# mittagessen/conformer_ocr

Measured on AMD Instinct MI355X. Metric: text lines/sec (whole node) + CER vs reference, 96×1200 bf16 batch, higher is better.
Workload: dtype bf16; 1 GPU; cfg2: conformer D=256 L=12 heads=4 sub_ch=256, batch 32 x 96x1200 per GPU, forward + CTC greedy; batches_in_queue=1, parallelism=1 independent rank(s), weights by one RCCL broadcast, streams_per_gpu=4, hipgraph_replay=True, launched_by=in-process, gpu_max_hw_queues=4, gpu_max_hw_queues_preset_by_caller=True

## Files before the change

### conformer_ocr_amd/build.py

```python
from __future__ import annotations

import os
import shutil
import subprocess
import sys

PKG = os.path.dirname(os.path.abspath(__file__))
CSRC = os.path.join(PKG, 'csrc')
LIB_DIR = os.path.join(PKG, 'lib')
LIB = os.path.join(LIB_DIR, 'libcocr_hip.so')
INCLUDE = os.path.join(os.path.dirname(PKG), 'include')
ARCH = 'gfx950'


def sources():
    srcs = [os.path.join(CSRC, f) for f in sorted(os.listdir(CSRC))]
    return srcs + [os.path.join(INCLUDE, 'cocr.h')]


def source_hash() -> str:
    import hashlib
    h = hashlib.sha256()
    for s in sources():
        h.update(os.path.basename(s).encode() + b'\0')
# ... 27 lines not shown
        i = cmd.index('-amdgpu-mfma-vgpr-form')
        cmd = cmd[:i - 1] + cmd[i + 1:]
        if verbose:
            print('retrying without -amdgpu-mfma-vgpr-form', flush=True)
        subprocess.check_call(cmd)


def build(force: bool = False, verbose: bool = True, out: str = None) -> str:
    if out is not None:
        return _build_to(out, verbose)
    if not force and up_to_date():
        return LIB
    return _build_to(LIB, verbose)


def _build_to(LIB: str, verbose: bool) -> str:
    hipcc = shutil.which('hipcc') or '/opt/rocm/bin/hipcc'
    if not os.path.exists(hipcc):
        raise RuntimeError('hipcc not found: cannot build libcocr_hip.so')
    os.makedirs(LIB_DIR, exist_ok=True)
    src_hash = source_hash()
    obj_dir = os.path.join(LIB_DIR, 'obj', src_hash)
    os.makedirs(obj_dir, exist_ok=True)
    flags = [f'--offload-arch={ARCH}', '-O3', '-std=c++17', '-fPIC', '-fno-gpu-rdc', '-mllvm', '-amdgpu-mfma-vgpr-form',
             '-Wall', '-Wno-unused-function', f'-DCOCR_SRC_HASH="{src_hash}"', '-I', INCLUDE]
    flags[0:0] = os.environ.get('COCR_HIPCC_FLAGS', '').split()
    units = [f for f in sorted(os.listdir(CSRC)) if f.endswith('.hip')]
    objs = [os.path.join(obj_dir, u[:-4] + '.o') for u in units]
    jobs = [([hipcc] + flags + ['-c', os.path.join(CSRC, u), '-o', o], verbose) for u, o in zip(units, objs)]
    from concurrent.futures import ThreadPoolExecutor
    with ThreadPoolExecutor(max_workers=min(len(jobs), os.cpu_count() or 1)) as pool:
        list(pool.map(_compile, jobs))
    link = [hipcc, f'--offload-arch={ARCH}', '-shared', '-fPIC', '-fno-gpu-rdc'] + objs + ['-o', LIB + '.tmp']
    if verbose:
        print(' '.join(link), flush=True)
    subprocess.check_call(link)
    os.replace(LIB + '.tmp', LIB)
    with open(LIB + '.srchash.tmp', 'w') as fp:
        fp.write(src_hash + '\n')
    os.replace(LIB + '.srchash.tmp', LIB + '.srchash')
    for d in os.listdir(os.path.join(LIB_DIR, 'obj')):
# ... 9 lines not shown
```

### conformer_ocr_amd/csrc/attention.hip.h

```cpp
#pragma once
#include "common.hip.h"

__device__ __forceinline__ int xcd_remap_i(int bid, int nwg) {
    const int q = nwg >> 3, r = nwg & 7, xcd = bid & 7;
    return (xcd < r ? xcd * (q + 1) : r * (q + 1) + (xcd - r) * q) + (bid >> 3);
}

__device__ __forceinline__ float max3_f(float a, float b, float c) {
    float r;
    asm("v_max3_f32 %0, %1, %2, %3" : "=v"(r) : "v"(a), "v"(b), "v"(c));
    return r;
}

#define COCR_MFMA_WAIT "s_nop 7\n\ts_nop 7\n\ts_nop 3"
__device__ __forceinline__ void mfma_results_fence(f32x4 (&a)[4]) { asm volatile(COCR_MFMA_WAIT : "+v"(a[0]), "+v"(a[1]), "+v"(a[2]), "+v"(a[3])); }
__device__ __forceinline__ void mfma_results_fence(f32x4 (&a)[4], f32x4 (&b)[4]) {
    asm volatile(COCR_MFMA_WAIT : "+v"(a[0]), "+v"(a[1]), "+v"(a[2]), "+v"(a[3]), "+v"(b[0]), "+v"(b[1]), "+v"(b[2]), "+v"(b[3]));
}
__device__ __forceinline__ void mfma_results_fence(f32x4 (&a)[4], f32x4 (&b)[4], f32x4 (&c)[4]) {
    asm volatile(COCR_MFMA_WAIT : "+v"(a[0]), "+v"(a[1]), "+v"(a[2]), "+v"(a[3]), "+v"(b[0]), "+v"(b[1]), "+v"(b[2]), "+v"(b[3]), "+v"(c[0]), "+v"(c[1]), "+v"(c[2]),
                 "+v"(c[3]));
}

#ifndef COCR_ATT_EXP
// ... 421 lines not shown
constexpr int AF_SK = 20;
#ifndef COCR_AF_TWOPART
#define COCR_AF_TWOPART 1
#endif
constexpr int AF_WAVES = 8;
constexpr int AF_SROWS = 32;
constexpr size_t AF_LDS = (size_t)(2 * AF_TK + 16 * AF_QT + AF_TK) * 128 + AF_WAVES * AF_SROWS * AF_SK * sizeof(float);
static_assert(AF_LDS <= 160 * 1024, "LDS of the resident attention kernel");

struct AttnFullState {
    bf16x8 qu[2][2], qv[2][2];
    f32x4 o[2][4], osum[2];
    float m_run[2];
};

template <int NT>
__device__ __forceinline__ void attn_full_tiles(const unsigned char *ks, const unsigned char *vs, const unsigned char *ps, float *sk,
                                                AttnFullState &st, int lb_first, int Tn, int Tk, int kg0, int lane, bool sync_after_first = false) {
    typedef bf16_t T;
    constexpr int KC = 2, DT = 4, RS = 128;
    const int il = lane & 15, g = lane >> 4;
    const int fo0 = ((g ^ (il & 7)) << 4), fo1 = (((4 + g) ^ (il & 7)) << 4);
    auto &qu = st.qu;
    auto &qv = st.qv;
    auto &o = st.o;
    auto &osum = st.osum;
    auto &m_run = st.m_run;
    bf16x8 ones;
#pragma unroll
    for (int j = 0; j < 8; ++j) ones[j] = il == 0 ? (T)1.0f : (T)0.0f;
// ... 83 lines not shown
#pragma unroll
        for (int t = 0; t < NT; ++t) { const float x = __shfl_xor(tmax[t], 16, 64); tmax[t] = max3_f(tmax[t], x, x); }
#pragma unroll
        for (int t = 0; t < NT; ++t) { const float x = __shfl_xor(tmax[t], 32, 64); tmax[t] = max3_f(tmax[t], x, x); }
        constexpr float LAZY = 8.0f;
        bool need[NT], any = first_tile;
#pragma unroll
        for (int t = 0; t < NT; ++t) { need[t] = first_tile || __builtin_amdgcn_ballot_w64(tmax[t] > LAZY) != 0; any = any || need[t]; }
        if (any) {
#pragma unroll
            for (int t = 0; t < NT; ++t) {
                const float delta = first_tile ? tmax[t] : (need[t] ? fmaxf(tmax[t], 0.f) : 0.f);
                const float alpha = first_tile ? 1.0f : __builtin_amdgcn_exp2f(-delta);
                m_run[t] = first_tile ? tmax[t] : m_run[t] + delta;
#pragma unroll
                for (int r = 0; r < 4; ++r) osum[t][r] *= alpha;
#pragma unroll
                for (int d = 0; d < DT; ++d)
#pragma unroll
                    for (int r = 0; r < 4; ++r) o[t][d][r] *= alpha;
#pragma unroll
                for (int tt = 0; tt < 4; ++tt)
#pragma unroll
                    for (int r = 0; r < 4; ++r) sc[t][tt][r] -= delta;
            }
        }
#pragma unroll
        for (int t = 0; t < NT; ++t) {
#pragma unroll
            for (int tt = 0; tt < 4; ++tt)
#pragma unroll
                for (int r = 0; r < 4; ++r) pb[t][tt >> 1][4 * (tt & 1) + r] = (T)__builtin_amdgcn_exp2f(sc[t][tt][r]);
            osum[t] = mma16(ones, pb[t][0], osum[t]);
            osum[t] = mma16(ones, pb[t][1], osum[t]);
        }
#pragma unroll
        for (int d = 0; d < DT; ++d) {
            const bf16x8 v0 = load_vt_frag<true>(vs, RS, j0, d, il, g, T()), v1 = load_vt_frag<true>(vs, RS, j0 + 32, d, il, g, T());
#pragma unroll
// ... 146 lines not shown
```

### conformer_ocr_amd/csrc/common.hip.h

```cpp
#pragma once
#include <hip/hip_runtime.h>
#include <stdint.h>

typedef __attribute__((address_space(3))) void *lds_ptr_t;
typedef __attribute__((address_space(1))) const void *gbl_ptr_t;

typedef __bf16 bf16_t;
typedef __bf16 bf16x8 __attribute__((ext_vector_type(8)));
typedef __bf16 bf16x4 __attribute__((ext_vector_type(4)));
typedef __bf16 bf16x2 __attribute__((ext_vector_type(2)));
typedef float f32x2 __attribute__((ext_vector_type(2)));
typedef float f32x4 __attribute__((ext_vector_type(4)));
typedef float f32x8 __attribute__((ext_vector_type(8)));

#define COCR_WAVE 64

template <typename T> struct FragOf;
template <> struct FragOf<bf16_t> { typedef bf16x8 type; };
template <> struct FragOf<float> { typedef f32x8 type; };

__device__ __forceinline__ f32x4 mma16(const bf16x8 &a, const bf16x8 &b, f32x4 c) {
    return __builtin_amdgcn_mfma_f32_16x16x32_bf16(a, b, c, 0, 0, 0);
}
__device__ __forceinline__ f32x4 mma16(const f32x8 &a, const f32x8 &b, f32x4 c) {
// ... 9 lines not shown
}
template <typename T> __device__ __forceinline__ typename FragOf<T>::type zero_frag() {
    typename FragOf<T>::type z;
#pragma unroll
    for (int j = 0; j < 8; ++j) z[j] = (T)0.0f;
    return z;
}

__device__ __forceinline__ float to_f32(float x) { return x; }
__device__ __forceinline__ float to_f32(bf16_t x) { return (float)x; }
template <typename T> __device__ __forceinline__ T from_f32(float x) { return (T)x; }

__device__ __forceinline__ float sigmoid_f(float x) { return __builtin_amdgcn_rcpf(1.0f + __expf(-x)); }
__device__ __forceinline__ float silu_f(float x) { return x * sigmoid_f(x); }

template <int CTRL, int ROW_MASK> __device__ __forceinline__ float dpp_f32(float v, float old) {
    return __builtin_bit_cast(float, __builtin_amdgcn_update_dpp(__builtin_bit_cast(int, old), __builtin_bit_cast(int, v), CTRL, ROW_MASK, 0xF, false));
}
__device__ __forceinline__ float wave_sum(float v) {
    v += dpp_f32<0xB1, 0xF>(v, 0.f);
    v += dpp_f32<0x4E, 0xF>(v, 0.f);
    v += dpp_f32<0x141, 0xF>(v, 0.f);
    v += dpp_f32<0x140, 0xF>(v, 0.f);
    v += dpp_f32<0x142, 0xA>(v, 0.f);
    v += dpp_f32<0x143, 0xC>(v, 0.f);
    return __builtin_bit_cast(float, __builtin_amdgcn_readlane(__builtin_bit_cast(int, v), 63));
}
__device__ __forceinline__ float wave_max(float v) {
    v = fmaxf(v, dpp_f32<0xB1, 0xF>(v, v));
    v = fmaxf(v, dpp_f32<0x4E, 0xF>(v, v));
// ... 10 lines not shown
```

### conformer_ocr_amd/csrc/rowchain.hip.h

```cpp
#pragma once
#include <type_traits>

#include "gemm.hip.h"
#include "rowchain_args.hip.h"

#ifndef COCR_STAMP_WG
#define COCR_STAMP_WG 7
#endif
#ifndef COCR_RC_EXP
#define COCR_RC_EXP 0
#endif

__device__ __forceinline__ void swap32(float &a, float &b) { asm("s_nop 1\n\tv_permlane32_swap_b32 %0, %1" : "+v"(a), "+v"(b)); }
__device__ __forceinline__ void swap16(float &a, float &b) { asm("s_nop 1\n\tv_permlane16_swap_b32 %0, %1" : "+v"(a), "+v"(b)); }
__device__ __forceinline__ float butterfly4(float a, float b, float c, float d) {
    swap32(a, b);
    swap32(c, d);
    float ab = a + b, cd = c + d;
    swap16(ab, cd);
    return ab + cd;
}

__device__ __forceinline__ int xcd_remap_rows(int bid, int nwg) {
    const int q = nwg >> 3, r = nwg & 7, xcd = bid & 7;
    return (xcd < r ? xcd * (q + 1) : r * (q + 1) + (xcd - r) * q) + (bid >> 3);
}

#ifndef COCR_RC_PAIR
#define COCR_RC_PAIR 0
#endif
template <int D, int MT> constexpr bool rowchain_pair_form() { return COCR_RC_PAIR && D == 256 && MT == 3; }

template <int D, int MT> constexpr size_t rowchain_slack_bytes() { return rowchain_pair_form<D, MT>() ? 2048 : 4096; }
template <int D, int MT> constexpr size_t rowchain_lds_bytes() {
    return (size_t)(D / 64) * 16 * MT * 128 + 2 * 4 * (size_t)(16 * MT) * 128 + rowchain_slack_bytes<D, MT>() + 16 * (size_t)D + 12 * (size_t)(16 * MT) + 64;
}
template <int D, int MT> constexpr int rowchain_dw_pass() { return rowchain_pair_form<D, MT>() ? 128 : 256; }
template <int D, int MT, int DWK> constexpr int rowchain_taps_place() {
    if (DWK == 0 || (DWK + 1) % 8 != 0) return 0;
    constexpr size_t cw = rowchain_dw_pass<D, MT>(), rpi = 64 / (cw / 8);
    constexpr size_t hsb = 2 * 4 * (size_t)(16 * MT) * 128 + rowchain_slack_bytes<D, MT>(), win = ((16 * MT + DWK - 1 + rpi - 1) / rpi) * 1024, taps = (size_t)(DWK + 1) * cw * 4;
    if (win + taps <= hsb) return 1;
    if (rowchain_pair_form<D, MT>()) return 0;
    if (rowchain_lds_bytes<D, MT>() + taps <= 160 * 1024) return 2;
// ... 20 lines not shown
    constexpr int PANEL = BMC * 128;
    constexpr int IMGX = (D / 64) * PANEL;
    constexpr int IMGH = 4 * PANEL;
    constexpr int OS = 256 * 2 + 16;
    constexpr int OSD = D * 2 + 16;
    constexpr int SLICE = 16 * 512;
    constexpr int PROW = 80;
    constexpr int HSB = 2 * IMGH + (int)rowchain_slack_bytes<D, MT>();
    extern __shared__ __attribute__((aligned(16))) unsigned char smem[];
    unsigned char *xa = smem;
    unsigned char *hs = smem + IMGX;
    float *lnp = reinterpret_cast<float *>(smem + IMGX + HSB);
    long long *rowoff = reinterpret_cast<long long *>(smem + IMGX + HSB + 16 * D);
    int *tpos = reinterpret_cast<int *>(smem + IMGX + HSB + 16 * D + 8 * BMC);

    const int tid = threadIdx.x, lane = tid & 63;
    const int wave = __builtin_amdgcn_readfirstlane(tid >> 6);
    const int r16 = lane & 15, g = lane >> 4, swz = r16 & 7;
    const int rblk = p.xcd_order ? xcd_remap_rows(blockIdx.x, gridDim.x) : (int)blockIdx.x;
    const int M = p.M, m0 = rblk * BMC, mend = min(M, m0 + BMC);
    const int lrow = lane >> 3, cpos = lane & 7;
#ifdef COCR_CHAIN_STAMPS_BUILD
    int sk = 0;
#define RSTAMP() { if (p.stamps && rblk == COCR_STAMP_WG && lane == 0) p.stamps[wave * 64 + sk] = __builtin_readcyclecounter(); ++sk; }
#else
#define RSTAMP()
#endif
    RSTAMP()
    auto lds_fence_barrier = [&]() {
        asm volatile("s_waitcnt lgkmcnt(0)" ::: "memory");
// ... 68 lines not shown
    };
    RSTAMP()
    dw_taps(0);
    RSTAMP()
    constexpr int RING = rowchain_pair_form<D, MT>() ? 8 : 16;
    bf16x8 ring[RING];
    auto fill = [&](const T *slice, int f) { ring[f % RING] = *reinterpret_cast<const bf16x8 *>(slice + f * 512 + lane * 8); };
    const T *cur_run = p.st[0].W + (size_t)wave * (FRONT0 ? p.st[0].K / 256 : KS) * SLICE;
    {
#pragma unroll
        for (int f = 0; f < RING; ++f) fill(cur_run, f);
    }
    __builtin_amdgcn_sched_barrier(0);
    RSTAMP()
    f32x4 xs[MT][NJ];
    const size_t xblk = ((size_t)rblk * 8 + wave) * (MT * NJ) * 256 + lane * 4;
    auto load_stream = [&]() {
        if (p.x_in_blocked) {
#pragma unroll
            for (int i = 0; i < MT; ++i)
#pragma unroll
                for (int c = 0; c < NJ; ++c) {
                    if constexpr (COCR_RC_EXP & 1) xs[i][c] = (f32x4){(float)r16, 1.f, (float)g, 0.5f};
                    else xs[i][c] = *reinterpret_cast<const f32x4 *>(p.x + xblk + (i * NJ + c) * 256);
                }
            return;
        }
#pragma unroll
        for (int i = 0; i < MT; ++i) {
            const float *xrow = p.x + (size_t)min(m0 + 16 * i + r16, mend - 1) * D + 32 * wave + 4 * g;
#pragma unroll
            for (int c = 0; c < NJ; ++c) {
                if constexpr (COCR_RC_EXP & 1) xs[i][c] = (f32x4){(float)r16, 1.f, (float)g, 0.5f};
                else xs[i][c] = *reinterpret_cast<const f32x4 *>(xrow + 256 * (c >> 1) + 16 * (c & 1));
            }
        }
    };
    constexpr int EARLY_XS = (DWK == 0 && !FRONT0) ? MT * NJ : 0;
    if constexpr (DWK == 0 && !FRONT0) load_stream();
    __builtin_amdgcn_sched_barrier(0);
    if (tid < BMC) {
        const int m = min(m0 + tid, M - 1), b = m / p.T_, t = m - b * p.T_;
        rowoff[tid] = ((long long)b * p.heads * p.Tp + t) * p.dhp;
        tpos[tid] = t;
    }
// ... 73 lines not shown
                        }
                    }
                }
#pragma unroll
                for (int i = 0; i < G; ++i) {
                    const int row = rb + i, cc = h * CW + c;
                    const bf16x2 o = (COCR_RC_EXP & 16384) ? (bf16x2){(T)acc[i][0], (T)acc[i][1]} : (bf16x2){(T)silu_f(acc[i][0]), (T)silu_f(acc[i][1])};
                    *reinterpret_cast<bf16x2 *>(xa + (cc >> 6) * PANEL + row * 128 + ((((cc & 63) >> 3) ^ (row & 7)) << 4) + (cc & 7) * 2) = o;
                    if constexpr (TAPS) {
                        if (p.tap_dw && m0 + row < mend) *reinterpret_cast<bf16x2 *>(p.tap_dw + (size_t)(m0 + row) * D + cc) = o;
                    }
                }
            }
            lds_fence_barrier();
        }
        load_stream();
        __builtin_amdgcn_sched_barrier(0);
        RSTAMP()
    }

    auto step = [&](const unsigned char *img, auto &acc, int c0, const T *nxt, auto &&side, auto FRESH, auto KKC) {
        constexpr bool fresh = decltype(FRESH)::value;
        constexpr int KK = decltype(KKC)::value;
#pragma unroll
        for (int kk = 0; kk < KK; ++kk) {
            constexpr int HT = MT > 3 ? MT / 2 : MT;
#pragma unroll
            for (int h0 = 0; h0 < MT; h0 += HT) {
                bf16x8 a[HT];
#pragma unroll
                for (int i = 0; i < HT; ++i) {
// ... 21 lines not shown
                    fill(nxt, 2 * (kk & 3));
                    fill(nxt, 2 * (kk & 3) + 1);
                }
            }
            side(kk);
            __builtin_amdgcn_sched_barrier(0);
        }
        if constexpr (KK < (RING == 16 ? 8 : 4) && !(COCR_RC_EXP & 128)) {
#pragma unroll
            for (int f = 2 * KK; f < RING; ++f) fill(nxt, f);
            __builtin_amdgcn_sched_barrier(0);
        }
        cur_run = nxt;
    };
    auto no_side = [](int) {};
    auto request_ln_params = [&](const ChainStage &st) {
        if (wave < 4) {
            const float *src = wave == 0 ? st.g1 : wave == 1 ? st.b1 : wave == 2 ? (st.g2 ? st.g2 : st.g1) : (st.b2 ? st.b2 : st.b1);
#pragma unroll
            for (int c = 0; c < D / 256; ++c)
                __builtin_amdgcn_global_load_lds((gbl_ptr_t)(src + c * 256 + lane * 4), (lds_ptr_t)(reinterpret_cast<unsigned char *>(lnp) + wave * D * 4 + c * 1024), 16, 0, 0);
        }
    };
    struct Bias2 { f32x4 v[2]; };
    auto load_bias = [&](const float *bias) {
        Bias2 b;
        b.v[0] = *reinterpret_cast<const f32x4 *>(bias + 32 * wave + 4 * g);
        b.v[1] = *reinterpret_cast<const f32x4 *>(bias + 32 * wave + 16 + 4 * g);
        return b;
    };
    auto add_bias_to_stream = [&](const float *bias, float alpha) {
#pragma unroll
        for (int ns = 0; ns < NS; ++ns) {
            const Bias2 b = load_bias(bias + 256 * ns);
#pragma unroll
            for (int j = 0; j < 2; ++j)
#pragma unroll
                for (int i = 0; i < MT; ++i) xs[i][2 * ns + j] += b.v[j] * alpha;
        }
    };
    auto store_stream = [&](float *dst) {
        if constexpr (COCR_RC_EXP & 2) { asm volatile("" :: "v"(xs[0][0][0])); return; }
        if (dst == p.x && p.x_out_blocked) {
#pragma unroll
            for (int i = 0; i < MT; ++i)
#pragma unroll
                for (int c = 0; c < NJ; ++c) *reinterpret_cast<f32x4 *>(dst + xblk + (i * NJ + c) * 256) = xs[i][c];
            return;
        }
#pragma unroll
        for (int i = 0; i < MT; ++i) {
            if (m0 + 16 * i + r16 < mend) {
                float *xrow = dst + (size_t)(m0 + 16 * i + r16) * D + 32 * wave + 4 * g;
#pragma unroll
                for (int c = 0; c < NJ; ++c) *reinterpret_cast<f32x4 *>(xrow + 256 * (c >> 1) + 16 * (c & 1)) = xs[i][c];
            }
        }
    };
    auto row_stats = [&](unsigned char *pbuf, bool wait_params, float (&mean)[MT], float (&rstd)[MT]) {
        if constexpr (COCR_RC_EXP & 32) { for (int i = 0; i < MT; ++i) { mean[i] = 0.f; rstd[i] = 1.f; } lds_fence_barrier(); return; }
        float s[MT], ss[MT];
#pragma unroll
        for (int i = 0; i < MT; ++i) {
            f32x4 a = xs[i][0], b = xs[i][0] * xs[i][0];
#pragma unroll
            for (int c = 1; c < NJ; ++c) { a += xs[i][c]; b = __builtin_elementwise_fma(xs[i][c], xs[i][c], b); }
            s[i] = (a[0] + a[1]) + (a[2] + a[3]);
            ss[i] = (b[0] + b[1]) + (b[2] + b[3]);
        }
#pragma unroll
        for (int i0 = 0; i0 < MT; i0 += 4) {
            const int i1 = min(i0 + 1, MT - 1), i2 = min(i0 + 2, MT - 1), i3 = min(i0 + 3, MT - 1);
            const float ts = butterfly4(s[i0], s[i1], s[i2], s[i3]), tss = butterfly4(ss[i0], ss[i1], ss[i2], ss[i3]);
            const int tile = g == 0 ? i0 : g == 1 ? i2 : g == 2 ? i1 : i3;
            *reinterpret_cast<f32x2 *>(pbuf + (16 * tile + r16) * PROW + wave * 8) = (f32x2){ts, tss};
        }
        if (wait_params && wave < 4) {
            if constexpr (KD == 8 && KL == 8) asm volatile("s_waitcnt vmcnt(%0)" :: "n"(RING) : "memory");
            else asm volatile("s_waitcnt vmcnt(0)" ::: "memory");
        }
        lds_fence_barrier();
        const float inv_d = p.inv_d;
#pragma unroll
        for (int i = 0; i < MT; ++i) {
            const unsigned char *pr = pbuf + (16 * i + r16) * PROW;
            f32x4 v = *reinterpret_cast<const f32x4 *>(pr);
            if constexpr (!(COCR_RC_EXP & 4)) {
#pragma unroll
                for (int w2 = 1; w2 < 4; ++w2) v += *reinterpret_cast<const f32x4 *>(pr + 16 * w2);
            }
            const float S = v[0] + v[2], SS = v[1] + v[3];
            mean[i] = S * inv_d;
            const float ex2 = SS * inv_d;
            rstd[i] = __builtin_amdgcn_rsqf(fmaxf(__builtin_fmaf(-mean[i], mean[i], ex2), 0.f) + 1e-5f);
        }
    };
    auto normalise = [&](int which, const float (&mean)[MT], const float (&rstd)[MT], auto IN_PLACE) {
        constexpr bool in_place = decltype(IN_PLACE)::value;
        if constexpr (COCR_RC_EXP & 8192) return;
        const float *ga = lnp + which * 2 * D, *be = ga + D;
#pragma unroll
        for (int c = 0; c < NJ; ++c) {
            const int col = 256 * (c >> 1) + 32 * wave + 16 * (c & 1) + 4 * g;
            const f32x4 gv = *reinterpret_cast<const f32x4 *>(ga + col), bv = *reinterpret_cast<const f32x4 *>(be + col);
#pragma unroll
            for (int i = 0; i < MT; ++i) {
                const float r = rstd[i], mr = -mean[i] * r;
                const f32x4 y = __builtin_elementwise_fma(__builtin_elementwise_fma(xs[i][c], (f32x4){r, r, r, r}, (f32x4){mr, mr, mr, mr}), gv, bv);
                if constexpr (in_place) {
                    xs[i][c] = y;
                } else {
                    const int row = 16 * i + r16;
                    const bf16x4 o = {(T)y[0], (T)y[1], (T)y[2], (T)y[3]};
                    *reinterpret_cast<bf16x4 *>(xa + (col >> 6) * PANEL + row * 128 + ((((col & 63) >> 3) ^ (row & 7)) << 4) + (col & 4) * 2) = o;
                }
            }
        }
    };
    auto rowln_epilogue = [&](const ChainStage &st, unsigned char *pbuf) {
        const bool chained = st.g2 != nullptr;
        if constexpr (TAPS) { if (st.tap_pre) store_stream(st.tap_pre); }
        float mean[MT], rstd[MT];
        if (!chained) {
            if (st.store_x) store_stream(p.x);
            row_stats(pbuf, true, mean, rstd);
            normalise(0, mean, rstd, std::false_type{});
        } else {
            row_stats(pbuf, true, mean, rstd);
            normalise(0, mean, rstd, std::true_type{});
            if (st.store_x) store_stream(p.x);
            if constexpr (TAPS) { if (st.tap_post) store_stream(st.tap_post); }
            row_stats(pbuf + BMC * PROW, false, mean, rstd);
            normalise(1, mean, rstd, std::false_type{});
        }
        lds_fence_barrier();
        if (st.store_xn) {
            for (int id = tid; id < BMC * (D / 8); id += 512) {
                const int row = id / (D / 8), ch = id - row * (D / 8);
                if (m0 + row < mend)
                    copy16(p.xn + (size_t)(m0 + row) * D + ch * 8, reinterpret_cast<const T *>(xa + (ch >> 3) * PANEL + row * 128 + (((ch & 7) ^ (row & 7)) << 4)));
            }
        }
    };

    auto run_stage = [&](auto KIND, auto FIRST, const ChainStage &st, const T *after) {
        constexpr int kind = decltype(KIND)::value;
        if constexpr (kind == ST_ROWLN) {
            request_ln_params(st);
            auto slice = [&](int ns, int ks) { return st.W + ((size_t)(ns * 8 + wave) * KS + ks) * SLICE; };
            if constexpr (decltype(FIRST)::value) {
                f32x4 acc[MT][NJ];
#pragma unroll
                for (int ns = 0; ns < NS; ++ns)
#pragma unroll
                    for (int ks = 0; ks < KS; ++ks) {
                        const T *nxt = ks + 1 < KS ? slice(ns, ks + 1) : (ns + 1 < NS ? slice(ns + 1, 0) : after);
                        if (ks == 0) step(xa, acc, 2 * ns, nxt, no_side, std::true_type{}, KKR{});
                        else step(xa + ks * 4 * PANEL, acc, 2 * ns, nxt, no_side, std::false_type{}, KKR{});
                    }
                add_bias_to_stream(st.bias, 1.0f);
#pragma unroll
                for (int i = 0; i < MT; ++i)
#pragma unroll
                    for (int c = 0; c < NJ; ++c) xs[i][c] += acc[i][c];
            } else {
                add_bias_to_stream(st.bias, 1.0f);
#pragma unroll
                for (int ns = 0; ns < NS; ++ns)
#pragma unroll
                    for (int ks = 0; ks < KS; ++ks)
                        step(xa + ks * 4 * PANEL, xs, 2 * ns, ks + 1 < KS ? slice(ns, ks + 1) : (ns + 1 < NS ? slice(ns + 1, 0) : after), no_side, std::false_type{}, KKR{});
            }
            RSTAMP()
            rowln_epilogue(st, hs);
            RSTAMP()
        } else if constexpr (kind == ST_FRONT) {
            static_assert(decltype(FIRST)::value, "FRONT is a first stage");
            request_ln_params(st);
            const int nsl = st.K / 256;
            auto slice = [&](int ns, int ks) { return st.W + ((size_t)(ns * 8 + wave) * nsl + ks) * SLICE; };
#pragma unroll
            for (int i = 0; i < MT; ++i)
#pragma unroll
                for (int c = 0; c < NJ; ++c) xs[i][c] = (f32x4){0.f, 0.f, 0.f, 0.f};
            add_bias_to_stream(st.bias, 1.0f);
#pragma unroll 1
            for (int ks = 0; ks < nsl; ++ks) {
                if (ks + 1 < nsl) front_dma(ks + 1);
                const unsigned char *img = hs + (ks & 1) * IMGH;
#pragma unroll
                for (int ns = 0; ns < NS; ++ns)
                    step(img, xs, 2 * ns, ns + 1 < NS ? slice(ns + 1, ks) : (ks + 1 < nsl ? slice(0, ks + 1) : after), no_side, std::false_type{}, KK8{});
                if (ks + 1 < nsl) {
                    asm volatile("s_waitcnt vmcnt(%0)" :: "n"(RING) : "memory");
                    lds_fence_barrier();
                }
            }
            RSTAMP()
            rowln_epilogue(st, hs + (nsl & 1) * IMGH);
            RSTAMP()
        } else if constexpr (kind == ST_FFN) {
            const int FF = st.N, nchunks = FF / 256;
            auto w1 = [&](int c, int ks) { return st.W + ((size_t)(c * 8 + wave) * KS + ks) * SLICE; };
            auto w2 = [&](int c, int ns) { return st.W2 + ((size_t)(ns * 8 + wave) * (FF / 32) + c * 8) * 1024; };
            f32x4 acc1[MT][2];
            Bias2 bb;
            auto silu_tile = [&](int tIdx, unsigned char *hb, auto PIN) {
                if constexpr (COCR_RC_EXP & 4096) return;
                const int i = tIdx >> 1, j = tIdx & 1;
                if constexpr (decltype(PIN)::value) asm volatile("" : "+v"(acc1[i][j]));
                const int jj = 32 * wave + 16 * j + 4 * g;
                const int ch16 = (jj & 63) >> 3, row = 16 * i + r16;
                typedef float f32x2_t __attribute__((ext_vector_type(2)));
                const f32x4 v4 = acc1[i][j] + bb.v[j];
                unsigned packed[2];
#pragma unroll
                for (int h = 0; h < 2; ++h) {
                    const f32x2_t v = {v4[2 * h], v4[2 * h + 1]};
                    f32x2_t e = v * (f32x2_t){-1.44269504088896340736f, -1.44269504088896340736f};
                    if constexpr (!(COCR_RC_EXP & 16)) e = (f32x2_t){__builtin_amdgcn_exp2f(e[0]), __builtin_amdgcn_exp2f(e[1])} + (f32x2_t){1.0f, 1.0f};
                    const f32x2_t o = (COCR_RC_EXP & 16) ? v * e : v * (f32x2_t){__builtin_amdgcn_rcpf(e[0]), __builtin_amdgcn_rcpf(e[1])};
                    packed[h] = __builtin_bit_cast(unsigned, __builtin_convertvector(o, bf16x2));
                }
                typedef unsigned u32x2_t __attribute__((ext_vector_type(2)));
                *reinterpret_cast<u32x2_t *>(hb + (jj >> 6) * PANEL + row * 128 + ((ch16 ^ (row & 7)) << 4) + ((jj & 7) >> 2) * 8) = (u32x2_t){packed[0], packed[1]};
            };
            auto p1 = [&](int c, const T *then) {
                if (wave >= 4) __builtin_amdgcn_s_setprio(1);
#pragma unroll
                for (int ks = 0; ks < KS; ++ks) {
                    if (ks == 0) step(xa, acc1, 0, KS > 1 ? w1(c, 1) : then, no_side, std::true_type{}, KKP1{});
                    else step(xa + ks * 4 * PANEL, acc1, 0, ks + 1 < KS ? w1(c, ks + 1) : then, no_side, std::false_type{}, KKP1{});
                }
                if (wave >= 4) __builtin_amdgcn_s_setprio(0);
            };
            request_ln_params(st);
            bb = load_bias(st.bias);
            p1(0, nchunks > 1 ? w1(1, 0) : w2(0, 0));
            RSTAMP()
#pragma unroll
            for (int t2 = 0; t2 < 2 * MT; ++t2) silu_tile(t2, hs, std::false_type{});
            add_bias_to_stream(st.bias2, st.alpha);
            RSTAMP()
            lds_fence_barrier();
            RSTAMP()
            for (int c = 1; c < nchunks; ++c) {
                bb = load_bias(st.bias + c * 256);
                p1(c, w2(c - 1, 0));
                RSTAMP()
                unsigned char *hb = hs + (c & 1) * IMGH;
#pragma unroll
                for (int ns = 0; ns < NS; ++ns)
                    step(hs + ((c - 1) & 1) * IMGH, xs, 2 * ns, ns + 1 < NS ? w2(c - 1, ns + 1) : (c + 1 < nchunks ? w1(c + 1, 0) : w2(c, 0)),
                         [&](int kk) {
#pragma unroll
                             for (int t2 = 0; t2 < 2 * MT; ++t2) if ((t2 * 8 * NS) / (2 * MT) == ns * 8 + kk) silu_tile(t2, hb, std::true_type{});
                         }, std::false_type{}, KK8{});
                RSTAMP()
                lds_fence_barrier();
                RSTAMP()
            }
#pragma unroll
            for (int ns = 0; ns < NS; ++ns)
                step(hs + ((nchunks - 1) & 1) * IMGH, xs, 2 * ns, ns + 1 < NS ? w2(nchunks - 1, ns + 1) : after, no_side, std::false_type{}, KKL{});
            RSTAMP()
            rowln_epilogue(st, hs + (nchunks & 1) * IMGH);
            RSTAMP()
        } else if constexpr (kind == ST_GLU) {
            EpiGLU<T> e{st.out, D, st.bias, 2 * D};
            auto slice = [&](int s2, int ks) { return st.W + ((size_t)(s2 * 8 + wave) * KS + ks) * SLICE; };
            constexpr int NSTEP = 2 * D / 256;
#pragma unroll 1
            for (int s2 = 0; s2 < NSTEP; ++s2) {
                const Bias2 bb = load_bias(st.bias + s2 * 256);
                f32x4 acc[MT][2];
#pragma unroll
                for (int ks = 0; ks < KS; ++ks) {
                    const T *nxt = ks + 1 < KS ? slice(s2, ks + 1) : (s2 + 1 < NSTEP ? slice(s2 + 1, 0) : after);
                    if (ks == 0) step(xa, acc, 0, nxt, no_side, std::true_type{}, KKG{});
                    else step(xa + ks * 4 * PANEL, acc, 0, nxt, no_side, std::false_type{}, KKG{});
                }
#pragma unroll
                for (int i = 0; i < MT; ++i) {
                    const int row = 16 * i + r16;
                    bf16x4 o;
#pragma unroll
                    for (int q = 0; q < 4; ++q) o[q] = (T)((acc[i][0][q] + bb.v[0][q]) * sigmoid_f(acc[i][1][q] + bb.v[1][q]));
                    *reinterpret_cast<bf16x4 *>(hs + row * OSD + (s2 * 128 + 16 * wave + 4 * g) * 2) = o;
                }
            }
            lds_fence_barrier();
            for (int id = tid; id < BMC * (D / 8); id += 512) {
                const int row = id / (D / 8), ch = id - row * (D / 8);
                if (m0 + row < mend) e.store(m0 + row, ch * 8, reinterpret_cast<const T *>(hs + row * OSD + ch * 16), 8);
            }
        } else if constexpr (kind == ST_QKV) {
            auto slice = [&](int s3, int ks) { return st.W + ((size_t)(s3 * 8 + wave) * KS + ks) * SLICE; };
            constexpr int NSTEP = 3 * D / 256;
#pragma unroll
            for (int s3 = 0; s3 < NSTEP; ++s3) {
                const Bias2 bb = load_bias(st.bias + s3 * 256);
                f32x4 acc[MT][2];
#pragma unroll
                for (int ks = 0; ks < KS; ++ks) {
                    const T *nxt = ks + 1 < KS ? slice(s3, ks + 1) : (s3 + 1 < NSTEP ? slice(s3 + 1, 0) : after);
                    if (ks == 0) step(xa, acc, 0, nxt, no_side, std::true_type{}, KKQ{});
                    else step(xa + ks * 4 * PANEL, acc, 0, nxt, no_side, std::false_type{}, KKQ{});
                }
                unsigned char *tile = hs + (s3 & 1) * (BMC * OS);
                if constexpr (COCR_RC_EXP & 1024) { asm volatile("" :: "v"(acc[0][0]), "v"(acc[MT - 1][1])); continue; }
#pragma unroll
                for (int j = 0; j < 2; ++j)
#pragma unroll
                    for (int i = 0; i < MT; ++i) {
                        const int row = 16 * i + r16;
                        bf16x4 o;
#pragma unroll
                        for (int q = 0; q < 4; ++q) o[q] = (T)(acc[i][j][q] + bb.v[j][q]);
                        *reinterpret_cast<bf16x4 *>(tile + row * OS + (32 * wave + 16 * j + 4 * g) * 2) = o;
                    }
                RSTAMP()
                lds_fence_barrier();
                {
                    const int which = s3 / NS;
                    T *base = which == 0 ? st.q : (which == 1 ? st.k : st.v);
                    const int ch = tid & 31, hd = (s3 - which * NS) * 256 + ch * 8, hh = hd / p.dh, d = hd - hh * p.dh;
                    base += (size_t)hh * p.Tp * p.dhp + d;
#pragma unroll
                    for (int i = 0; i < MT; ++i) {
                        const int row = (tid >> 5) + 16 * i;
                        if (m0 + row < mend) copy16(base + rowoff[row], reinterpret_cast<const T *>(tile + row * OS + ch * 16));
                    }
                }
            }
        }
    };
    auto first_slice = [&](int i) -> const T * { return p.st[i].W + (size_t)wave * ((i == 0 && FRONT0) ? p.st[0].K / 256 : KS) * SLICE; };
    run_stage(std::integral_constant<int, K0>{}, std::true_type{}, p.st[0], K1 >= 0 ? first_slice(1) : first_slice(0));
    run_stage(std::integral_constant<int, K1>{}, std::false_type{}, p.st[1], K2 >= 0 ? first_slice(2) : first_slice(0));
    run_stage(std::integral_constant<int, K2>{}, std::false_type{}, p.st[2], K3 >= 0 ? first_slice(3) : first_slice(0));
    run_stage(std::integral_constant<int, K3>{}, std::false_type{}, p.st[3], first_slice(0));
    RSTAMP()
#undef RSTAMP
}

template <int D, int MT, int DWK, int K0, int K1, int K2, int K3, bool TAPS, int KD = 8, int KL = 8>
static inline hipError_t launch_rowchain_mt(hipStream_t s, const ChainArgs &a) {
    constexpr size_t lds = rowchain_lds_bytes<D, MT>() + (rowchain_taps_place<D, MT, DWK>() == 2 ? (size_t)(DWK + 1) * 1024 : 0);
    static_assert(lds <= 160 * 1024, "LDS of one workgroup");
    auto kern = rowchain_kernel<D, MT, DWK, K0, K1, K2, K3, TAPS, KD, KL>;
    hipError_t e = raise_lds_limit((const void *)kern, lds);
    if (e != hipSuccess) return e;
    hipLaunchKernelGGL(kern, dim3(ceil_div(a.M, 16 * MT)), dim3(512), lds, s, a);
    return hipGetLastError();
}

// ... 44 lines not shown
```

Measured before the change: 34620 lines/s.

## Cut register pressure in rowchain by rereading kernargs and overlapping stream loads

The rowchain kernel now re-reads arguments through the kernarg segment pointer instead of holding them in registers, and recomputes lane-derived indices behind opaque asm so they are not kept live. In the first ROWLN stage, the residual stream load and bias fetch move into the first MFMA step so they overlap the GEMM. LN parameter DMA uses an inline asm that the compiler does not count. Scalar inline-asm add/mul/sub helpers replace vector ops in the SiLU epilogue and the attention rescale to stop packed-op formation. The aim is lower VGPR/SGPR pressure and better latency hiding, at the cost of extra scalar loads and fragile uncounted DMA ordering.

```diff
diff --git a/conformer_ocr_amd/build.py b/conformer_ocr_amd/build.py
--- a/conformer_ocr_amd/build.py
+++ b/conformer_ocr_amd/build.py
@@ -65,6 +65,13 @@
     return _build_to(LIB, verbose)
 
 
+def compile_flags(src_hash: str) -> list:
+    flags = [f'--offload-arch={ARCH}', '-O3', '-std=c++17', '-fPIC', '-fno-gpu-rdc', '-mllvm', '-amdgpu-mfma-vgpr-form',
+             '-Wall', '-Wno-unused-function', f'-DCOCR_SRC_HASH="{src_hash}"', '-I', INCLUDE]
+    flags[0:0] = os.environ.get('COCR_HIPCC_FLAGS', '').split()
+    return flags
+
+
 def _build_to(LIB: str, verbose: bool) -> str:
     hipcc = shutil.which('hipcc') or '/opt/rocm/bin/hipcc'
     if not os.path.exists(hipcc):
@@ -73,9 +80,7 @@
     src_hash = source_hash()
     obj_dir = os.path.join(LIB_DIR, 'obj', src_hash)
     os.makedirs(obj_dir, exist_ok=True)
-    flags = [f'--offload-arch={ARCH}', '-O3', '-std=c++17', '-fPIC', '-fno-gpu-rdc', '-mllvm', '-amdgpu-mfma-vgpr-form',
-             '-Wall', '-Wno-unused-function', f'-DCOCR_SRC_HASH="{src_hash}"', '-I', INCLUDE]
-    flags[0:0] = os.environ.get('COCR_HIPCC_FLAGS', '').split()
+    flags = compile_flags(src_hash)
     units = [f for f in sorted(os.listdir(CSRC)) if f.endswith('.hip')]
     objs = [os.path.join(obj_dir, u[:-4] + '.o') for u in units]
     jobs = [([hipcc] + flags + ['-c', os.path.join(CSRC, u), '-o', o], verbose) for u, o in zip(units, objs)]
diff --git a/conformer_ocr_amd/csrc/attention.hip.h b/conformer_ocr_amd/csrc/attention.hip.h
--- a/conformer_ocr_amd/csrc/attention.hip.h
+++ b/conformer_ocr_amd/csrc/attention.hip.h
@@ -459,6 +459,9 @@
     float m_run[2];
 };
 
+#ifndef COCR_ATT_PK
+#define COCR_ATT_PK 0
+#endif
 template <int NT>
 __device__ __forceinline__ void attn_full_tiles(const unsigned char *ks, const unsigned char *vs, const unsigned char *ps, float *sk,
                                                 AttnFullState &st, int lb_first, int Tn, int Tk, int kg0, int lane, bool sync_after_first = false) {
@@ -572,15 +575,15 @@
                 const float alpha = first_tile ? 1.0f : __builtin_amdgcn_exp2f(-delta);
                 m_run[t] = first_tile ? tmax[t] : m_run[t] + delta;
 #pragma unroll
-                for (int r = 0; r < 4; ++r) osum[t][r] *= alpha;
+                for (int r = 0; r < 4; ++r) osum[t][r] = COCR_ATT_PK ? osum[t][r] * alpha : mul1_f32(osum[t][r], alpha);
 #pragma unroll
                 for (int d = 0; d < DT; ++d)
 #pragma unroll
-                    for (int r = 0; r < 4; ++r) o[t][d][r] *= alpha;
+                    for (int r = 0; r < 4; ++r) o[t][d][r] = COCR_ATT_PK ? o[t][d][r] * alpha : mul1_f32(o[t][d][r], alpha);
 #pragma unroll
                 for (int tt = 0; tt < 4; ++tt)
 #pragma unroll
-                    for (int r = 0; r < 4; ++r) sc[t][tt][r] -= delta;
+                    for (int r = 0; r < 4; ++r) sc[t][tt][r] = COCR_ATT_PK ? sc[t][tt][r] - delta : sub1_f32(sc[t][tt][r], delta);
             }
         }
 #pragma unroll
diff --git a/conformer_ocr_amd/csrc/common.hip.h b/conformer_ocr_amd/csrc/common.hip.h
--- a/conformer_ocr_amd/csrc/common.hip.h
+++ b/conformer_ocr_amd/csrc/common.hip.h
@@ -47,6 +47,12 @@
 __device__ __forceinline__ float sigmoid_f(float x) { return __builtin_amdgcn_rcpf(1.0f + __expf(-x)); }
 __device__ __forceinline__ float silu_f(float x) { return x * sigmoid_f(x); }
 
+__device__ __forceinline__ float add1_f32(float a, float b) { float r; asm("v_add_f32 %0, %1, %2" : "=v"(r) : "v"(a), "v"(b)); return r; }
+__device__ __forceinline__ float mul1_f32(float a, float b) { float r; asm("v_mul_f32 %0, %1, %2" : "=v"(r) : "v"(a), "v"(b)); return r; }
+__device__ __forceinline__ float mul1_f32_s(float s, float b) { float r; asm("v_mul_f32 %0, %1, %2" : "=v"(r) : "s"(s), "v"(b)); return r; }
+__device__ __forceinline__ float sub1_f32(float a, float b) { float r; asm("v_sub_f32 %0, %1, %2" : "=v"(r) : "v"(a), "v"(b)); return r; }
+__device__ __forceinline__ float inc1_f32(float a) { float r; asm("v_add_f32 %0, 1.0, %1" : "=v"(r) : "v"(a)); return r; }
+
 template <int CTRL, int ROW_MASK> __device__ __forceinline__ float dpp_f32(float v, float old) {
     return __builtin_bit_cast(float, __builtin_amdgcn_update_dpp(__builtin_bit_cast(int, old), __builtin_bit_cast(int, v), CTRL, ROW_MASK, 0xF, false));
 }
diff --git a/conformer_ocr_amd/csrc/rowchain.hip.h b/conformer_ocr_amd/csrc/rowchain.hip.h
--- a/conformer_ocr_amd/csrc/rowchain.hip.h
+++ b/conformer_ocr_amd/csrc/rowchain.hip.h
@@ -21,6 +21,11 @@
     return ab + cd;
 }
 
+__device__ __forceinline__ void lds_dma16_uncounted(const void *gsrc, unsigned lds_dst) {
+    unsigned keep;
+    asm volatile("s_mov_b32 %0, m0\n\ts_mov_b32 m0, %2\n\ts_nop 0\n\tglobal_load_lds_dwordx4 %1, off\n\ts_mov_b32 m0, %0" : "=&s"(keep) : "v"(gsrc), "s"(lds_dst) : "memory");
+}
+
 __device__ __forceinline__ int xcd_remap_rows(int bid, int nwg) {
     const int q = nwg >> 3, r = nwg & 7, xcd = bid & 7;
     return (xcd < r ? xcd * (q + 1) : r * (q + 1) + (xcd - r) * q) + (bid >> 3);
@@ -28,6 +33,9 @@
 
 #ifndef COCR_RC_PAIR
 #define COCR_RC_PAIR 0
+#endif
+#ifndef COCR_RC_PK_SILU
+#define COCR_RC_PK_SILU 0
 #endif
 template <int D, int MT> constexpr bool rowchain_pair_form() { return COCR_RC_PAIR && D == 256 && MT == 3; }
 
@@ -78,6 +86,13 @@
     long long *rowoff = reinterpret_cast<long long *>(smem + IMGX + HSB + 16 * D);
     int *tpos = reinterpret_cast<int *>(smem + IMGX + HSB + 16 * D + 8 * BMC);
 
+    typedef const __attribute__((address_space(4))) ChainArgs KArgs;
+    typedef const __attribute__((address_space(4))) ChainStage KStage;
+    auto args = [&]() -> KArgs & {
+        KArgs *k = (KArgs *)__builtin_amdgcn_kernarg_segment_ptr();
+        asm volatile("" : "+s"(k));
+        return *k;
+    };
     const int tid = threadIdx.x, lane = tid & 63;
     const int wave = __builtin_amdgcn_readfirstlane(tid >> 6);
     const int r16 = lane & 15, g = lane >> 4, swz = r16 & 7;
@@ -176,21 +191,27 @@
     __builtin_amdgcn_sched_barrier(0);
     RSTAMP()
     f32x4 xs[MT][NJ];
-    const size_t xblk = ((size_t)rblk * 8 + wave) * (MT * NJ) * 256 + lane * 4;
+    auto lane_now = [&]() { unsigned l = lane; asm volatile("" : "+v"(l)); return l; };
+    const size_t xblk_wave = ((size_t)rblk * 8 + wave) * (MT * NJ) * 256;
+    auto xblk_lane = [&]() { return lane_now() * 4u; };
     auto load_stream = [&]() {
-        if (p.x_in_blocked) {
+        if (args().x_in_blocked) {
+            const float *xb = args().x + xblk_wave;
+            const unsigned xl = xblk_lane();
 #pragma unroll
             for (int i = 0; i < MT; ++i)
 #pragma unroll
                 for (int c = 0; c < NJ; ++c) {
                     if constexpr (COCR_RC_EXP & 1) xs[i][c] = (f32x4){(float)r16, 1.f, (float)g, 0.5f};
-                    else xs[i][c] = *reinterpret_cast<const f32x4 *>(p.x + xblk + (i * NJ + c) * 256);
+                    else xs[i][c] = *reinterpret_cast<const f32x4 *>(xb + xl + (i * NJ + c) * 256);
                 }
             return;
         }
+        const float *xbase = args().x + (size_t)m0 * D + 32 * wave;
+        const unsigned ln = lane_now(), lr = ln & 15, lg = ln >> 4;
 #pragma unroll
         for (int i = 0; i < MT; ++i) {
-            const float *xrow = p.x + (size_t)min(m0 + 16 * i + r16, mend - 1) * D + 32 * wave + 4 * g;
+            const float *xrow = xbase + ((unsigned)min(16 * i + (int)lr, mend - 1 - m0) * D + 4 * lg);
 #pragma unroll
             for (int c = 0; c < NJ; ++c) {
                 if constexpr (COCR_RC_EXP & 1) xs[i][c] = (f32x4){(float)r16, 1.f, (float)g, 0.5f};
@@ -294,7 +315,6 @@
             }
             lds_fence_barrier();
         }
-        load_stream();
         __builtin_amdgcn_sched_barrier(0);
         RSTAMP()
     }
@@ -346,44 +366,57 @@
         cur_run = nxt;
     };
     auto no_side = [](int) {};
-    auto request_ln_params = [&](const ChainStage &st) {
+    auto request_ln_params = [&](KStage &st) {
         if (wave < 4) {
-            const float *src = wave == 0 ? st.g1 : wave == 1 ? st.b1 : wave == 2 ? (st.g2 ? st.g2 : st.g1) : (st.b2 ? st.b2 : st.b1);
+            const float *g1 = st.g1, *b1 = st.b1, *g2 = st.g2, *b2 = st.b2;
+            const float *ga = (wave & 2) && g2 ? g2 : g1, *be = (wave & 2) && b2 ? b2 : b1;
+            const float *src = (wave & 1) ? be : ga;
 #pragma unroll
             for (int c = 0; c < D / 256; ++c)
-                __builtin_amdgcn_global_load_lds((gbl_ptr_t)(src + c * 256 + lane * 4), (lds_ptr_t)(reinterpret_cast<unsigned char *>(lnp) + wave * D * 4 + c * 1024), 16, 0, 0);
+                lds_dma16_uncounted(src + c * 256 + lane * 4, (unsigned)(size_t)(lds_ptr_t)(reinterpret_cast<unsigned char *>(lnp) + wave * D * 4 + c * 1024));
         }
     };
     struct Bias2 { f32x4 v[2]; };
     auto load_bias = [&](const float *bias) {
         Bias2 b;
-        b.v[0] = *reinterpret_cast<const f32x4 *>(bias + 32 * wave + 4 * g);
-        b.v[1] = *reinterpret_cast<const f32x4 *>(bias + 32 * wave + 16 + 4 * g);
+        const float *bw = bias + 32 * wave;
+        const unsigned go = 4 * (lane_now() >> 4);
+        b.v[0] = *reinterpret_cast<const f32x4 *>(bw + go);
+        b.v[1] = *reinterpret_cast<const f32x4 *>(bw + go + 16);
         return b;
     };
-    auto add_bias_to_stream = [&](const float *bias, float alpha) {
-#pragma unroll
-        for (int ns = 0; ns < NS; ++ns) {
-            const Bias2 b = load_bias(bias + 256 * ns);
+    struct BiasD { Bias2 b[NS]; };
+    auto load_bias_d = [&](const float *bias) {
+        BiasD b;
+#pragma unroll
+        for (int ns = 0; ns < NS; ++ns) b.b[ns] = load_bias(bias + 256 * ns);
+        return b;
+    };
+    auto add_bias_to_stream = [&](const BiasD &b, float alpha) {
+#pragma unroll
+        for (int ns = 0; ns < NS; ++ns)
 #pragma unroll
             for (int j = 0; j < 2; ++j)
 #pragma unroll
-                for (int i = 0; i < MT; ++i) xs[i][2 * ns + j] += b.v[j] * alpha;
-        }
+                for (int i = 0; i < MT; ++i) xs[i][2 * ns + j] += b.b[ns].v[j] * alpha;
     };
     auto store_stream = [&](float *dst) {
         if constexpr (COCR_RC_EXP & 2) { asm volatile("" :: "v"(xs[0][0][0])); return; }
-        if (dst == p.x && p.x_out_blocked) {
+        if (dst == args().x && args().x_out_blocked) {
+            float *xb = dst + xblk_wave;
+            const unsigned xl = xblk_lane();
 #pragma unroll
             for (int i = 0; i < MT; ++i)
 #pragma unroll
-                for (int c = 0; c < NJ; ++c) *reinterpret_cast<f32x4 *>(dst + xblk + (i * NJ + c) * 256) = xs[i][c];
+                for (int c = 0; c < NJ; ++c) *reinterpret_cast<f32x4 *>(xb + xl + (i * NJ + c) * 256) = xs[i][c];
             return;
         }
+        float *xbase = dst + (size_t)m0 * D + 32 * wave;
+        const unsigned ln = lane_now(), lr = ln & 15, lg = ln >> 4;
 #pragma unroll
         for (int i = 0; i < MT; ++i) {
-            if (m0 + 16 * i + r16 < mend) {
-                float *xrow = dst + (size_t)(m0 + 16 * i + r16) * D + 32 * wave + 4 * g;
+            if (m0 + 16 * i + (int)lr < mend) {
+                float *xrow = xbase + ((16 * i + lr) * D + 4 * lg);
 #pragma unroll
                 for (int c = 0; c < NJ; ++c) *reinterpret_cast<f32x4 *>(xrow + 256 * (c >> 1) + 16 * (c & 1)) = xs[i][c];
             }
@@ -412,10 +445,11 @@
             else asm volatile("s_waitcnt vmcnt(0)" ::: "memory");
         }
         lds_fence_barrier();
-        const float inv_d = p.inv_d;
+        const int lrow16 = lane_now() & 15;
+        const float inv_d = args().inv_d;
 #pragma unroll
         for (int i = 0; i < MT; ++i) {
-            const unsigned char *pr = pbuf + (16 * i + r16) * PROW;
+            const unsigned char *pr = pbuf + (16 * i + lrow16) * PROW;
             f32x4 v = *reinterpret_cast<const f32x4 *>(pr);
             if constexpr (!(COCR_RC_EXP & 4)) {
 #pragma unroll
@@ -431,9 +465,10 @@
         constexpr bool in_place = decltype(IN_PLACE)::value;
         if constexpr (COCR_RC_EXP & 8192) return;
         const float *ga = lnp + which * 2 * D, *be = ga + D;
+        const int lg = lane_now() >> 4, lr = lane_now() & 15;
 #pragma unroll
         for (int c = 0; c < NJ; ++c) {
-            const int col = 256 * (c >> 1) + 32 * wave + 16 * (c & 1) + 4 * g;
+            const int col = 256 * (c >> 1) + 32 * wave + 16 * (c & 1) + 4 * lg;
             const f32x4 gv = *reinterpret_cast<const f32x4 *>(ga + col), bv = *reinterpret_cast<const f32x4 *>(be + col);
 #pragma unroll
             for (int i = 0; i < MT; ++i) {
@@ -442,61 +477,69 @@
                 if constexpr (in_place) {
                     xs[i][c] = y;
                 } else {
-                    const int row = 16 * i + r16;
+                    const int row = 16 * i + lr;
                     const bf16x4 o = {(T)y[0], (T)y[1], (T)y[2], (T)y[3]};
                     *reinterpret_cast<bf16x4 *>(xa + (col >> 6) * PANEL + row * 128 + ((((col & 63) >> 3) ^ (row & 7)) << 4) + (col & 4) * 2) = o;
                 }
             }
         }
     };
-    auto rowln_epilogue = [&](const ChainStage &st, unsigned char *pbuf) {
-        const bool chained = st.g2 != nullptr;
-        if constexpr (TAPS) { if (st.tap_pre) store_stream(st.tap_pre); }
+    auto rowln_epilogue = [&](auto &&st, unsigned char *pbuf) {
+        const bool chained = st().g2 != nullptr;
+        if constexpr (TAPS) { if (st().tap_pre) store_stream(st().tap_pre); }
         float mean[MT], rstd[MT];
         if (!chained) {
-            if (st.store_x) store_stream(p.x);
+            if (st().store_x) store_stream(args().x);
             row_stats(pbuf, true, mean, rstd);
             normalise(0, mean, rstd, std::false_type{});
         } else {
             row_stats(pbuf, true, mean, rstd);
             normalise(0, mean, rstd, std::true_type{});
-            if (st.store_x) store_stream(p.x);
-            if constexpr (TAPS) { if (st.tap_post) store_stream(st.tap_post); }
+            if (st().store_x) store_stream(args().x);
+            if constexpr (TAPS) { if (st().tap_post) store_stream(st().tap_post); }
             row_stats(pbuf + BMC * PROW, false, mean, rstd);
             normalise(1, mean, rstd, std::false_type{});
         }
         lds_fence_barrier();
-        if (st.store_xn) {
+        if (st().store_xn) {
             for (int id = tid; id < BMC * (D / 8); id += 512) {
                 const int row = id / (D / 8), ch = id - row * (D / 8);
                 if (m0 + row < mend)
-                    copy16(p.xn + (size_t)(m0 + row) * D + ch * 8, reinterpret_cast<const T *>(xa + (ch >> 3) * PANEL + row * 128 + (((ch & 7) ^ (row & 7)) << 4)));
-            }
-        }
-    };
-
-    auto run_stage = [&](auto KIND, auto FIRST, const ChainStage &st, const T *after) {
+                    copy16(args().xn + (size_t)(m0 + row) * D + ch * 8, reinterpret_cast<const T *>(xa + (ch >> 3) * PANEL + row * 128 + (((ch & 7) ^ (row & 7)) << 4)));
+            }
+        }
+    };
+
+    auto run_stage = [&](auto KIND, auto FIRST, auto SI, const T *after) {
         constexpr int kind = decltype(KIND)::value;
+        auto st = [&]() -> KStage & { return args().st[decltype(SI)::value]; };
         if constexpr (kind == ST_ROWLN) {
-            request_ln_params(st);
-            auto slice = [&](int ns, int ks) { return st.W + ((size_t)(ns * 8 + wave) * KS + ks) * SLICE; };
+            request_ln_params(st());
+            const T *W = st().W;
+            auto slice = [&](int ns, int ks) { return W + ((size_t)(ns * 8 + wave) * KS + ks) * SLICE; };
             if constexpr (decltype(FIRST)::value) {
                 f32x4 acc[MT][NJ];
+                BiasD bv;
+                if constexpr (DWK == 0) bv = load_bias_d(st().bias);
+                else __builtin_amdgcn_s_waitcnt(0x0F70);
 #pragma unroll
                 for (int ns = 0; ns < NS; ++ns)
 #pragma unroll
                     for (int ks = 0; ks < KS; ++ks) {
                         const T *nxt = ks + 1 < KS ? slice(ns, ks + 1) : (ns + 1 < NS ? slice(ns + 1, 0) : after);
-                        if (ks == 0) step(xa, acc, 2 * ns, nxt, no_side, std::true_type{}, KKR{});
-                        else step(xa + ks * 4 * PANEL, acc, 2 * ns, nxt, no_side, std::false_type{}, KKR{});
+                        auto side = [&](int kk) {
+                            if constexpr (DWK != 0) { if (ns == 0 && ks == 0 && kk == 0) { load_stream(); bv = load_bias_d(st().bias); } }
+                        };
+                        if (ks == 0) step(xa, acc, 2 * ns, nxt, side, std::true_type{}, KKR{});
+                        else step(xa + ks * 4 * PANEL, acc, 2 * ns, nxt, side, std::false_type{}, KKR{});
                     }
-                add_bias_to_stream(st.bias, 1.0f);
+                add_bias_to_stream(bv, 1.0f);
 #pragma unroll
                 for (int i = 0; i < MT; ++i)
 #pragma unroll
                     for (int c = 0; c < NJ; ++c) xs[i][c] += acc[i][c];
             } else {
-                add_bias_to_stream(st.bias, 1.0f);
+                add_bias_to_stream(load_bias_d(st().bias), 1.0f);
 #pragma unroll
                 for (int ns = 0; ns < NS; ++ns)
 #pragma unroll
@@ -508,14 +551,15 @@
             RSTAMP()
         } else if constexpr (kind == ST_FRONT) {
             static_assert(decltype(FIRST)::value, "FRONT is a first stage");
-            request_ln_params(st);
-            const int nsl = st.K / 256;
-            auto slice = [&](int ns, int ks) { return st.W + ((size_t)(ns * 8 + wave) * nsl + ks) * SLICE; };
+            request_ln_params(st());
+            const int nsl = st().K / 256;
+            const T *W = st().W;
+            auto slice = [&](int ns, int ks) { return W + ((size_t)(ns * 8 + wave) * nsl + ks) * SLICE; };
 #pragma unroll
             for (int i = 0; i < MT; ++i)
 #pragma unroll
                 for (int c = 0; c < NJ; ++c) xs[i][c] = (f32x4){0.f, 0.f, 0.f, 0.f};
-            add_bias_to_stream(st.bias, 1.0f);
+            add_bias_to_stream(load_bias_d(st().bias), 1.0f);
 #pragma unroll 1
             for (int ks = 0; ks < nsl; ++ks) {
                 if (ks + 1 < nsl) front_dma(ks + 1);
@@ -532,9 +576,11 @@
             rowln_epilogue(st, hs + (nsl & 1) * IMGH);
             RSTAMP()
         } else if constexpr (kind == ST_FFN) {
-            const int FF = st.N, nchunks = FF / 256;
-            auto w1 = [&](int c, int ks) { return st.W + ((size_t)(c * 8 + wave) * KS + ks) * SLICE; };
-            auto w2 = [&](int c, int ns) { return st.W2 + ((size_t)(ns * 8 + wave) * (FF / 32) + c * 8) * 1024; };
+            const int FF = st().N, nchunks = FF / 256;
+            const T *W1 = st().W, *W2 = st().W2;
+            const float *bias1 = st().bias;
+            auto w1 = [&](int c, int ks) { return W1 + ((size_t)(c * 8 + wave) * KS + ks) * SLICE; };
+            auto w2 = [&](int c, int ns) { return W2 + ((size_t)(ns * 8 + wave) * (FF / 32) + c * 8) * 1024; };
             f32x4 acc1[MT][2];
             Bias2 bb;
             auto silu_tile = [&](int tIdx, unsigned char *hb, auto PIN) {
@@ -544,8 +590,19 @@
                 const int jj = 32 * wave + 16 * j + 4 * g;
                 const int ch16 = (jj & 63) >> 3, row = 16 * i + r16;
                 typedef float f32x2_t __attribute__((ext_vector_type(2)));
+                unsigned packed[2];
+                if constexpr (decltype(PIN)::value && !(COCR_RC_EXP & 16) && !COCR_RC_PK_SILU) {
+                    float o[4];
+#pragma unroll
+                    for (int q = 0; q < 4; ++q) {
+                        const float v = add1_f32(acc1[i][j][q], bb.v[j][q]);
+                        const float e = inc1_f32(__builtin_amdgcn_exp2f(mul1_f32_s(-1.44269504088896340736f, v)));
+                        o[q] = mul1_f32(v, __builtin_amdgcn_rcpf(e));
+                    }
+#pragma unroll
+                    for (int h = 0; h < 2; ++h) packed[h] = __builtin_bit_cast(unsigned, __builtin_convertvector((f32x2_t){o[2 * h], o[2 * h + 1]}, bf16x2));
+                } else {
                 const f32x4 v4 = acc1[i][j] + bb.v[j];
-                unsigned packed[2];
 #pragma unroll
                 for (int h = 0; h < 2; ++h) {
                     const f32x2_t v = {v4[2 * h], v4[2 * h + 1]};
@@ -554,6 +611,7 @@
                     const f32x2_t o = (COCR_RC_EXP & 16) ? v * e : v * (f32x2_t){__builtin_amdgcn_rcpf(e[0]), __builtin_amdgcn_rcpf(e[1])};
                     packed[h] = __builtin_bit_cast(unsigned, __builtin_convertvector(o, bf16x2));
                 }
+                }
                 typedef unsigned u32x2_t __attribute__((ext_vector_type(2)));
                 *reinterpret_cast<u32x2_t *>(hb + (jj >> 6) * PANEL + row * 128 + ((ch16 ^ (row & 7)) << 4) + ((jj & 7) >> 2) * 8) = (u32x2_t){packed[0], packed[1]};
             };
@@ -566,18 +624,19 @@
                 }
                 if (wave >= 4) __builtin_amdgcn_s_setprio(0);
             };
-            request_ln_params(st);
-            bb = load_bias(st.bias);
+            request_ln_params(st());
+            bb = load_bias(bias1);
+            const BiasD b2v = load_bias_d(st().bias2);
             p1(0, nchunks > 1 ? w1(1, 0) : w2(0, 0));
             RSTAMP()
 #pragma unroll
             for (int t2 = 0; t2 < 2 * MT; ++t2) silu_tile(t2, hs, std::false_type{});
-            add_bias_to_stream(st.bias2, st.alpha);
+            add_bias_to_stream(b2v, st().alpha);
             RSTAMP()
             lds_fence_barrier();
             RSTAMP()
             for (int c = 1; c < nchunks; ++c) {
-                bb = load_bias(st.bias + c * 256);
+                bb = load_bias(bias1 + c * 256);
                 p1(c, w2(c - 1, 0));
                 RSTAMP()
                 unsigned char *hb = hs + (c & 1) * IMGH;
@@ -599,12 +658,13 @@
             rowln_epilogue(st, hs + (nchunks & 1) * IMGH);
             RSTAMP()
         } else if constexpr (kind == ST_GLU) {
-            EpiGLU<T> e{st.out, D, st.bias, 2 * D};
-            auto slice = [&](int s2, int ks) { return st.W + ((size_t)(s2 * 8 + wave) * KS + ks) * SLICE; };
+            const T *W = st().W;
+            const float *bias = st().bias;
+            auto slice = [&](int s2, int ks) { return W + ((size_t)(s2 * 8 + wave) * KS + ks) * SLICE; };
             constexpr int NSTEP = 2 * D / 256;
 #pragma unroll 1
             for (int s2 = 0; s2 < NSTEP; ++s2) {
-                const Bias2 bb = load_bias(st.bias + s2 * 256);
+                const Bias2 bb = load_bias(bias + s2 * 256);
                 f32x4 acc[MT][2];
 #pragma unroll
                 for (int ks = 0; ks < KS; ++ks) {
@@ -612,26 +672,30 @@
                     if (ks == 0) step(xa, acc, 0, nxt, no_side, std::true_type{}, KKG{});
                     else step(xa + ks * 4 * PANEL, acc, 0, nxt, no_side, std::false_type{}, KKG{});
                 }
+                const int lg = lane_now() >> 4, lr = lane_now() & 15;
 #pragma unroll
                 for (int i = 0; i < MT; ++i) {
-                    const int row = 16 * i + r16;
+                    const int row = 16 * i + lr;
                     bf16x4 o;
 #pragma unroll
                     for (int q = 0; q < 4; ++q) o[q] = (T)((acc[i][0][q] + bb.v[0][q]) * sigmoid_f(acc[i][1][q] + bb.v[1][q]));
-                    *reinterpret_cast<bf16x4 *>(hs + row * OSD + (s2 * 128 + 16 * wave + 4 * g) * 2) = o;
+                    *reinterpret_cast<bf16x4 *>(hs + row * OSD + (s2 * 128 + 16 * wave + 4 * lg) * 2) = o;
                 }
             }
             lds_fence_barrier();
+            EpiGLU<T> e{st().out, D, bias, 2 * D};
             for (int id = tid; id < BMC * (D / 8); id += 512) {
                 const int row = id / (D / 8), ch = id - row * (D / 8);
                 if (m0 + row < mend) e.store(m0 + row, ch * 8, reinterpret_cast<const T *>(hs + row * OSD + ch * 16), 8);
             }
         } else if constexpr (kind == ST_QKV) {
-            auto slice = [&](int s3, int ks) { return st.W + ((size_t)(s3 * 8 + wave) * KS + ks) * SLICE; };
+            const T *W = st().W;
+            const float *bias = st().bias;
+            auto slice = [&](int s3, int ks) { return W + ((size_t)(s3 * 8 + wave) * KS + ks) * SLICE; };
             constexpr int NSTEP = 3 * D / 256;
 #pragma unroll
             for (int s3 = 0; s3 < NSTEP; ++s3) {
-                const Bias2 bb = load_bias(st.bias + s3 * 256);
+                const Bias2 bb = load_bias(bias + s3 * 256);
                 f32x4 acc[MT][2];
 #pragma unroll
                 for (int ks = 0; ks < KS; ++ks) {
@@ -641,23 +705,25 @@
                 }
                 unsigned char *tile = hs + (s3 & 1) * (BMC * OS);
                 if constexpr (COCR_RC_EXP & 1024) { asm volatile("" :: "v"(acc[0][0]), "v"(acc[MT - 1][1])); continue; }
+                const int lg = lane_now() >> 4, lr = lane_now() & 15;
 #pragma unroll
                 for (int j = 0; j < 2; ++j)
 #pragma unroll
                     for (int i = 0; i < MT; ++i) {
-                        const int row = 16 * i + r16;
+                        const int row = 16 * i + lr;
                         bf16x4 o;
 #pragma unroll
                         for (int q = 0; q < 4; ++q) o[q] = (T)(acc[i][j][q] + bb.v[j][q]);
-                        *reinterpret_cast<bf16x4 *>(tile + row * OS + (32 * wave + 16 * j + 4 * g) * 2) = o;
+                        *reinterpret_cast<bf16x4 *>(tile + row * OS + (32 * wave + 16 * j + 4 * lg) * 2) = o;
                     }
                 RSTAMP()
                 lds_fence_barrier();
                 {
                     const int which = s3 / NS;
-                    T *base = which == 0 ? st.q : (which == 1 ? st.k : st.v);
-                    const int ch = tid & 31, hd = (s3 - which * NS) * 256 + ch * 8, hh = hd / p.dh, d = hd - hh * p.dh;
-                    base += (size_t)hh * p.Tp * p.dhp + d;
+                    T *base = which == 0 ? st().q : (which == 1 ? st().k : st().v);
+                    KArgs &pa = args();
+                    const int ch = tid & 31, hd = (s3 - which * NS) * 256 + ch * 8, hh = hd / pa.dh, d = hd - hh * pa.dh;
+                    base += (size_t)hh * pa.Tp * pa.dhp + d;
 #pragma unroll
                     for (int i = 0; i < MT; ++i) {
                         const int row = (tid >> 5) + 16 * i;
@@ -667,11 +733,15 @@
             }
         }
     };
-    auto first_slice = [&](int i) -> const T * { return p.st[i].W + (size_t)wave * ((i == 0 && FRONT0) ? p.st[0].K / 256 : KS) * SLICE; };
-    run_stage(std::integral_constant<int, K0>{}, std::true_type{}, p.st[0], K1 >= 0 ? first_slice(1) : first_slice(0));
-    run_stage(std::integral_constant<int, K1>{}, std::false_type{}, p.st[1], K2 >= 0 ? first_slice(2) : first_slice(0));
-    run_stage(std::integral_constant<int, K2>{}, std::false_type{}, p.st[2], K3 >= 0 ? first_slice(3) : first_slice(0));
-    run_stage(std::integral_constant<int, K3>{}, std::false_type{}, p.st[3], first_slice(0));
+    auto first_slice = [&](int i) -> const T * { KArgs &pa = args(); return pa.st[i].W + (size_t)wave * ((i == 0 && FRONT0) ? pa.st[0].K / 256 : KS) * SLICE; };
+    typedef std::integral_constant<int, 0> S0;
+    typedef std::integral_constant<int, 1> S1;
+    typedef std::integral_constant<int, 2> S2;
+    typedef std::integral_constant<int, 3> S3;
+    run_stage(std::integral_constant<int, K0>{}, std::true_type{}, S0{}, K1 >= 0 ? first_slice(1) : first_slice(0));
+    run_stage(std::integral_constant<int, K1>{}, std::false_type{}, S1{}, K2 >= 0 ? first_slice(2) : first_slice(0));
+    run_stage(std::integral_constant<int, K2>{}, std::false_type{}, S2{}, K3 >= 0 ? first_slice(3) : first_slice(0));
+    run_stage(std::integral_constant<int, K3>{}, std::false_type{}, S3{}, first_slice(0));
     RSTAMP()
 #undef RSTAMP
 }
```

Measured after the change: 28430 lines/s. -17.9%, worse.
